# jramapuram/BYOL

Measured on NVIDIA H100. Metric: images/sec, higher is better.
Workload: dtype bf16

## Files before the change

### byol_b200/csrc/common.cuh

```cuda
#pragma once
#include <cuda.h>
#include <cuda_bf16.h>
#include <cuda_runtime.h>
#include <stdint.h>

namespace byol {

typedef __nv_bfloat16 bf16;

void set_last_error(const char* fmt, ...);
int check_launch(const char* what);

static constexpr int kMaxDevices = 64;
int device_slot();
int device_sm_count();

int smem_opt_in(const void* kernel, int bytes, const char* what);

int tmap_bf16(CUtensorMap* tm, const void* base, int rank, const uint64_t* dims, const uint64_t* byte_strides,
              const uint32_t* box, CUtensorMapSwizzle swizzle, const char* what);
int tmap_2d(CUtensorMap* tm, const void* base, uint64_t rows, uint64_t cols, uint64_t ld, uint32_t box_rows,
            uint32_t box_cols, const char* what);

struct Fix128 {
  unsigned long long lo;
  long long hi;
  double spill;
};
static constexpr double kFixSplit = 1048576.0;
Fix128* fix_scratch(cudaStream_t stream, int64_t n);
int fix_done(cudaStream_t stream, int rc);
int fix_flush(Fix128* acc, float* dst, int64_t n, cudaStream_t stream);
int fix_flush_stats(Fix128* acc, float* col_sum, float* col_sqsum, int64_t n, cudaStream_t stream);

__device__ __forceinline__ void fix_add_words(Fix128* acc, unsigned long long lo, long long hi) {
  atomicAdd(&acc->lo, lo);
  atomicAdd(reinterpret_cast<unsigned long long*>(&acc->hi), (unsigned long long)hi);
}
__device__ __forceinline__ void fix_add(Fix128* acc, double v) {
  if (!(fabs(v) < kFixSplit)) {
    const double big = isfinite(v) ? trunc(v * 0x1p-20) * 0x1p20 : v;
    atomicAdd(&acc->spill, big);
    if (!isfinite(v)) return;
    v -= big;
  }
  const double x = v * 0x1p50;
  const double hi = floor(x * 0x1p-32);
  fix_add_words(acc, __double2ull_rn(x - hi * 0x1p32), (long long)hi);
}
__device__ __forceinline__ void fix_add_raw(Fix128* acc, const Fix128& v) {
  fix_add_words(acc, v.lo, v.hi);
  if (v.spill != 0.0) atomicAdd(&acc->spill, v.spill);
}
__host__ __device__ __forceinline__ double fix_value(const Fix128& a) {
  return ((double)a.hi * 0x1p-18 + (double)a.lo * 0x1p-50) + a.spill;
}

#define BYOL_CHECK_ARG(cond, ...)                 \
  do {                                            \
    if (!(cond)) {                                \
      ::byol::set_last_error(__VA_ARGS__);        \
      return -1;                                  \
    }                                             \
  } while (0)

__device__ __forceinline__ uint32_t smem_u32(const void* p) {
  return (uint32_t)__cvta_generic_to_shared(p);
}

__device__ __forceinline__ bool elect_one() {
  uint32_t pred = 0;
  asm volatile(
      "{\n"
      ".reg .b32 %%rx;\n"
      ".reg .pred %%px;\n"
      "elect.sync %%rx|%%px, %1;\n"
      "@%%px mov.s32 %0, 1;\n"
      "}\n"
      : "+r"(pred)
      : "r"(0xffffffffu));
  return pred != 0;
}

__device__ __forceinline__ float warp_sum(float v) {
#pragma unroll
  for (int o = 16; o > 0; o >>= 1) v += __shfl_xor_sync(0xffffffffu, v, o);
  return v;
}

__device__ __forceinline__ void mbar_init(uint64_t* bar, uint32_t count) {
  asm volatile("mbarrier.init.shared::cta.b64 [%0], %1;" ::"r"(smem_u32(bar)), "r"(count) : "memory");
}
__device__ __forceinline__ void fence_mbar_init() {
  asm volatile("fence.mbarrier_init.release.cluster;" ::: "memory");
}
__device__ __forceinline__ void mbar_arrive(uint64_t* bar) {
  asm volatile("mbarrier.arrive.shared::cta.b64 _, [%0];" ::"r"(smem_u32(bar)) : "memory");
}
__device__ __forceinline__ void mbar_arrive_expect_tx(uint64_t* bar, uint32_t bytes) {
  asm volatile("mbarrier.arrive.expect_tx.shared::cta.b64 _, [%0], %1;" ::"r"(smem_u32(bar)), "r"(bytes)
               : "memory");
// ... 98 lines not shown
        "{\n.reg .pred p;\nsetp.ne.b32 p, %98, 0;\n"
        "wgmma.mma_async.sync.aligned.m64n192k16.f32.bf16.bf16 {%0, %1, %2, %3, %4, %5, %6, %7, %8, %9, %10, %11, %12, %13, %14, %15, %16, %17, %18, %19, %20, %21, %22, %23, %24, %25, %26, %27, %28, %29, %30, %31, %32, %33, %34, %35, %36, %37, %38, %39, %40, %41, %42, %43, %44, %45, %46, %47, %48, %49, %50, %51, %52, %53, %54, %55, %56, %57, %58, %59, %60, %61, %62, %63, %64, %65, %66, %67, %68, %69, %70, %71, %72, %73, %74, %75, %76, %77, %78, %79, %80, %81, %82, %83, %84, %85, %86, %87, %88, %89, %90, %91, %92, %93, %94, %95}, %96, %97, p, 1, 1, %99, %100;\n}\n"
        : "+f"(d[0]), "+f"(d[1]), "+f"(d[2]), "+f"(d[3]), "+f"(d[4]), "+f"(d[5]), "+f"(d[6]), "+f"(d[7]), "+f"(d[8]), "+f"(d[9]), "+f"(d[10]), "+f"(d[11]), "+f"(d[12]), "+f"(d[13]), "+f"(d[14]), "+f"(d[15]), "+f"(d[16]), "+f"(d[17]), "+f"(d[18]), "+f"(d[19]), "+f"(d[20]), "+f"(d[21]), "+f"(d[22]), "+f"(d[23]), "+f"(d[24]), "+f"(d[25]), "+f"(d[26]), "+f"(d[27]), "+f"(d[28]), "+f"(d[29]), "+f"(d[30]), "+f"(d[31]), "+f"(d[32]), "+f"(d[33]), "+f"(d[34]), "+f"(d[35]), "+f"(d[36]), "+f"(d[37]), "+f"(d[38]), "+f"(d[39]), "+f"(d[40]), "+f"(d[41]), "+f"(d[42]), "+f"(d[43]), "+f"(d[44]), "+f"(d[45]), "+f"(d[46]), "+f"(d[47]), "+f"(d[48]), "+f"(d[49]), "+f"(d[50]), "+f"(d[51]), "+f"(d[52]), "+f"(d[53]), "+f"(d[54]), "+f"(d[55]), "+f"(d[56]), "+f"(d[57]), "+f"(d[58]), "+f"(d[59]), "+f"(d[60]), "+f"(d[61]), "+f"(d[62]), "+f"(d[63]), "+f"(d[64]), "+f"(d[65]), "+f"(d[66]), "+f"(d[67]), "+f"(d[68]), "+f"(d[69]), "+f"(d[70]), "+f"(d[71]), "+f"(d[72]), "+f"(d[73]), "+f"(d[74]), "+f"(d[75]), "+f"(d[76]), "+f"(d[77]), "+f"(d[78]), "+f"(d[79]), "+f"(d[80]), "+f"(d[81]), "+f"(d[82]), "+f"(d[83]), "+f"(d[84]), "+f"(d[85]), "+f"(d[86]), "+f"(d[87]), "+f"(d[88]), "+f"(d[89]), "+f"(d[90]), "+f"(d[91]), "+f"(d[92]), "+f"(d[93]), "+f"(d[94]), "+f"(d[95])
        : "l"(adesc), "l"(bdesc), "r"(accumulate), "n"(TA), "n"(TB));
  }
  if constexpr (N == 256) {
    asm volatile(
        "{\n.reg .pred p;\nsetp.ne.b32 p, %130, 0;\n"
        "wgmma.mma_async.sync.aligned.m64n256k16.f32.bf16.bf16 {%0, %1, %2, %3, %4, %5, %6, %7, %8, %9, %10, %11, %12, %13, %14, %15, %16, %17, %18, %19, %20, %21, %22, %23, %24, %25, %26, %27, %28, %29, %30, %31, %32, %33, %34, %35, %36, %37, %38, %39, %40, %41, %42, %43, %44, %45, %46, %47, %48, %49, %50, %51, %52, %53, %54, %55, %56, %57, %58, %59, %60, %61, %62, %63, %64, %65, %66, %67, %68, %69, %70, %71, %72, %73, %74, %75, %76, %77, %78, %79, %80, %81, %82, %83, %84, %85, %86, %87, %88, %89, %90, %91, %92, %93, %94, %95, %96, %97, %98, %99, %100, %101, %102, %103, %104, %105, %106, %107, %108, %109, %110, %111, %112, %113, %114, %115, %116, %117, %118, %119, %120, %121, %122, %123, %124, %125, %126, %127}, %128, %129, p, 1, 1, %131, %132;\n}\n"
        : "+f"(d[0]), "+f"(d[1]), "+f"(d[2]), "+f"(d[3]), "+f"(d[4]), "+f"(d[5]), "+f"(d[6]), "+f"(d[7]), "+f"(d[8]), "+f"(d[9]), "+f"(d[10]), "+f"(d[11]), "+f"(d[12]), "+f"(d[13]), "+f"(d[14]), "+f"(d[15]), "+f"(d[16]), "+f"(d[17]), "+f"(d[18]), "+f"(d[19]), "+f"(d[20]), "+f"(d[21]), "+f"(d[22]), "+f"(d[23]), "+f"(d[24]), "+f"(d[25]), "+f"(d[26]), "+f"(d[27]), "+f"(d[28]), "+f"(d[29]), "+f"(d[30]), "+f"(d[31]), "+f"(d[32]), "+f"(d[33]), "+f"(d[34]), "+f"(d[35]), "+f"(d[36]), "+f"(d[37]), "+f"(d[38]), "+f"(d[39]), "+f"(d[40]), "+f"(d[41]), "+f"(d[42]), "+f"(d[43]), "+f"(d[44]), "+f"(d[45]), "+f"(d[46]), "+f"(d[47]), "+f"(d[48]), "+f"(d[49]), "+f"(d[50]), "+f"(d[51]), "+f"(d[52]), "+f"(d[53]), "+f"(d[54]), "+f"(d[55]), "+f"(d[56]), "+f"(d[57]), "+f"(d[58]), "+f"(d[59]), "+f"(d[60]), "+f"(d[61]), "+f"(d[62]), "+f"(d[63]), "+f"(d[64]), "+f"(d[65]), "+f"(d[66]), "+f"(d[67]), "+f"(d[68]), "+f"(d[69]), "+f"(d[70]), "+f"(d[71]), "+f"(d[72]), "+f"(d[73]), "+f"(d[74]), "+f"(d[75]), "+f"(d[76]), "+f"(d[77]), "+f"(d[78]), "+f"(d[79]), "+f"(d[80]), "+f"(d[81]), "+f"(d[82]), "+f"(d[83]), "+f"(d[84]), "+f"(d[85]), "+f"(d[86]), "+f"(d[87]), "+f"(d[88]), "+f"(d[89]), "+f"(d[90]), "+f"(d[91]), "+f"(d[92]), "+f"(d[93]), "+f"(d[94]), "+f"(d[95]), "+f"(d[96]), "+f"(d[97]), "+f"(d[98]), "+f"(d[99]), "+f"(d[100]), "+f"(d[101]), "+f"(d[102]), "+f"(d[103]), "+f"(d[104]), "+f"(d[105]), "+f"(d[106]), "+f"(d[107]), "+f"(d[108]), "+f"(d[109]), "+f"(d[110]), "+f"(d[111]), "+f"(d[112]), "+f"(d[113]), "+f"(d[114]), "+f"(d[115]), "+f"(d[116]), "+f"(d[117]), "+f"(d[118]), "+f"(d[119]), "+f"(d[120]), "+f"(d[121]), "+f"(d[122]), "+f"(d[123]), "+f"(d[124]), "+f"(d[125]), "+f"(d[126]), "+f"(d[127])
        : "l"(adesc), "l"(bdesc), "r"(accumulate), "n"(TA), "n"(TB));
  }
}

template <int N>
__device__ __forceinline__ void acc_store_smem(float* buf, int ld, int row0, int col0, const float (&d)[N / 2]) {
  const int t = threadIdx.x & 127;
  const int r = row0 + (t >> 5) * 16 + ((t & 31) >> 2);
  const int c = col0 + 2 * (t & 3);
#pragma unroll
  for (int j = 0; j < N / 8; ++j) {
    *reinterpret_cast<float2*>(buf + (int64_t)r * ld + c + 8 * j) = make_float2(d[4 * j], d[4 * j + 1]);
    *reinterpret_cast<float2*>(buf + (int64_t)(r + 8) * ld + c + 8 * j) = make_float2(d[4 * j + 2], d[4 * j + 3]);
  }
}
__device__ __forceinline__ void acc_load_row32(const float* src, uint32_t (&r)[32]) {
#pragma unroll
  for (int j = 0; j < 8; ++j) {
    const uint4 q = *reinterpret_cast<const uint4*>(src + 4 * j);
    r[4 * j] = q.x; r[4 * j + 1] = q.y; r[4 * j + 2] = q.z; r[4 * j + 3] = q.w;
  }
}
__host__ __device__ constexpr int acc_ld(int cols) { return cols + 4; }

__device__ __forceinline__ uint64_t make_smem_desc_sw128(uint32_t smem_addr, uint32_t lbo_bytes,
                                                         uint32_t sbo_bytes) {
  uint64_t d = 0;
  d |= (uint64_t)((smem_addr & 0x3FFFFu) >> 4);
  d |= (uint64_t)((lbo_bytes >> 4) & 0x3FFFu) << 16;
  d |= (uint64_t)((sbo_bytes >> 4) & 0x3FFFu) << 32;
  d |= (uint64_t)1 << 62;
  return d;
}

__device__ __forceinline__ uint32_t sw128_offset(uint32_t row, uint32_t chunk) {
  return row * 128u + ((chunk ^ (row & 7u)) << 4);
}

__device__ __forceinline__ uint32_t pack_bf16x2(float lo, float hi) {
  __nv_bfloat162 v = __floats2bfloat162_rn(lo, hi);
  return *reinterpret_cast<uint32_t*>(&v);
}

__device__ __forceinline__ void bulk_load_1d(uint32_t dst_smem, const void* src, uint32_t bytes, uint64_t* bar) {
  asm volatile("cp.async.bulk.shared::cluster.global.mbarrier::complete_tx::bytes [%0], [%1], %2, [%3];" ::"r"(dst_smem),
               "l"(src), "r"(bytes), "r"(smem_u32(bar))
               : "memory");
}
__device__ __forceinline__ void tma_store_3d(const CUtensorMap* tmap, uint32_t src_smem, int c0, int c1, int c2) {
  asm volatile("cp.async.bulk.tensor.3d.global.shared::cta.bulk_group [%0, {%2, %3, %4}], [%1];" ::"l"(tmap),
               "r"(src_smem), "r"(c0), "r"(c1), "r"(c2)
               : "memory");
}

__device__ __forceinline__ uint64_t make_smem_desc_none(uint32_t smem_addr, uint32_t lbo_bytes, uint32_t sbo_bytes) {
  uint64_t d = 0;
  d |= (uint64_t)((smem_addr & 0x3FFFFu) >> 4);
  d |= (uint64_t)((lbo_bytes >> 4) & 0x3FFFu) << 16;
  d |= (uint64_t)((sbo_bytes >> 4) & 0x3FFFu) << 32;
  return d;
}

__device__ __forceinline__ uint64_t f2_pack(uint32_t lo, uint32_t hi) {
  uint64_t r;
  asm("mov.b64 %0, {%1, %2};" : "=l"(r) : "r"(lo), "r"(hi));
  return r;
}
__device__ __forceinline__ float2 f2_unpack(uint64_t v) {
  uint32_t lo, hi;
  asm("mov.b64 {%0, %1}, %2;" : "=r"(lo), "=r"(hi) : "l"(v));
  return make_float2(__uint_as_float(lo), __uint_as_float(hi));
}
__device__ __forceinline__ uint64_t f2_add(uint64_t a, uint64_t b) {
  const float2 x = f2_unpack(a), y = f2_unpack(b);
  return f2_pack(__float_as_uint(x.x + y.x), __float_as_uint(x.y + y.y));
}
__device__ __forceinline__ uint64_t f2_fma(uint64_t a, uint64_t b, uint64_t c) {
  const float2 x = f2_unpack(a), y = f2_unpack(b), z = f2_unpack(c);
  return f2_pack(__float_as_uint(fmaf(x.x, y.x, z.x)), __float_as_uint(fmaf(x.y, y.y, z.y)));
}
__device__ __forceinline__ uint32_t lds32(uint32_t addr) {
  uint32_t w;
  asm volatile("ld.shared.b32 %0, [%1];" : "=r"(w) : "r"(addr));
  return w;
}
__device__ __forceinline__ void stat_acc(uint32_t w, uint64_t& s1, uint64_t& s2) {
  const uint64_t x = f2_pack(w << 16, w & 0xffff0000u);
  s1 = f2_add(s1, x);
  s2 = f2_fma(x, x, s2);
}

__device__ __forceinline__ void stats_narrow(uint32_t stage_base, int lane, int rows_valid, uint64_t& s1,
                                             uint64_t& s2) {
  const uint32_t cp = (uint32_t)lane & 15u, rh = (uint32_t)lane >> 4;
  const uint32_t jc = cp >> 2, wq = cp & 3u;
  uint32_t offq[4];
// ... 20 lines not shown
```

### byol_b200/csrc/conv_igemm.cu

```cuda
#include <stdarg.h>
#include <stdio.h>
#include <stdlib.h>
#include <string.h>

#include "common.cuh"

namespace byol {

static constexpr int BM = 128;
static constexpr int BK = 64;
static constexpr int A_STAGE_BYTES = BM * 128;
static constexpr int GATHER_LAG = 2;

struct ConvGemmParams {
  const bf16* src;
  void* dst;
  const bf16* resid;
  const uint8_t* resid_mask;
  int resid_up;
  const float* resid_f32;
  const float* bias;
  float* col_sum;
  float* col_sqsum;
  Fix128* fx;
  int Nimg, Hs, Ws, C;
  int Ho, Wo;
  int KH, KW;
  int mul, base, dk, div;
  int M, Ndim, Kg;
  int ldc;
  int num_kb;
  int tiles_n;
  int out_fp32;
  int relu;
  int small_src;
  int fold;
  int parity;
  int Hh, Wh;
  int Mc;
  int ncls;
  int cls_list[4];
};

struct TileInfo {
  int m0, n0, nkb;
  int cls_idx, ph, pw, kh0, kw0, nkw;
};

template <bool GROUPED = false>
__device__ __forceinline__ TileInfo tile_info(const ConvGemmParams& p, int tile, int BN_) {
  TileInfo t;
  t.m0 = (tile / p.tiles_n) * BM;
  t.n0 = (tile % p.tiles_n) * BN_;
  t.nkb = p.num_kb;
  t.cls_idx = 0; t.ph = 0; t.pw = 0; t.kh0 = 0; t.kw0 = 0; t.nkw = p.KW;
  if (p.parity) {
    t.cls_idx = t.m0 / p.Mc;
    const int cls = p.cls_list[t.cls_idx];
    t.ph = cls >> 1;
    t.pw = cls & 1;
    t.kh0 = (t.ph + p.base) & 1;
    t.kw0 = (t.pw + p.base) & 1;
    const int nkh = (p.KH - t.kh0 + 1) >> 1;
    t.nkw = (p.KW - t.kw0 + 1) >> 1;
    t.nkb = nkh * t.nkw * (GROUPED ? 1 : p.C / BK);
  }
  return t;
}

template <int BN, int STAGES, bool A_TMA>
struct SmemLayout {
  static constexpr int EW = A_TMA ? 8 : 4;
  static constexpr int CPW = (BN / 32) / (EW / 4);
  static constexpr int NBUF = (A_TMA && BN == 128) ? 1 : 2;
  static constexpr int STAGE_PER_WARP = NBUF * 2048;
  static constexpr int B_STAGE_BYTES = BN * 128;
  static constexpr int A_OFF = 0;
  static constexpr int B_OFF = STAGES * A_STAGE_BYTES;
  static constexpr int STAGE_OUT_OFF = B_OFF + STAGES * B_STAGE_BYTES;
  static constexpr int ACC_LD = acc_ld(BN);
  static constexpr int ACC_OFF = STAGE_OUT_OFF + EW * STAGE_PER_WARP;
  static constexpr int BAR_OFF = ACC_OFF + BM * ACC_LD * 4;
  static constexpr int NEEDED = BAR_OFF + 256;
  static constexpr int TOTAL = NEEDED + 768;
  static_assert(TOTAL <= 232448, "one CTA per SM: <= 227 KB of dynamic shared memory");
};

static constexpr int IG_THREADS = 17 * 32;

template <int BN, int STAGES, bool A_TMA, bool GROUPED = false>
__global__ void __launch_bounds__(IG_THREADS, 1)
conv_igemm_kernel(const __grid_constant__ CUtensorMap tmapA, const __grid_constant__ CUtensorMap tmapB,
                  const __grid_constant__ CUtensorMap tmapC, const ConvGemmParams p, const int num_tiles) {
  static_assert(!GROUPED || (BN == 64 && !A_TMA), "grouped mode: 64-column tiles, gathered A operand");
  using L = SmemLayout<BN, STAGES, A_TMA>;
  constexpr int EW = L::EW;
  constexpr int CPW = L::CPW;
  constexpr int MMA_WARP = 8;
  constexpr int TMA_WARP = MMA_WARP + 8;
  extern __shared__ __align__(1024) uint8_t smem_raw[];
  uint8_t* smem = (uint8_t*)(((uintptr_t)smem_raw + 1023) & ~(uintptr_t)1023);
  if (smem + L::NEEDED > smem_raw + L::TOTAL) __trap();
  uint8_t* smemA = smem + L::A_OFF;
  uint8_t* smemB = smem + L::B_OFF;
  uint64_t* full_bar = (uint64_t*)(smem + L::BAR_OFF);
  uint64_t* empty_bar = full_bar + STAGES;
  uint64_t* tfull_bar = empty_bar + STAGES;
  uint64_t* tempty_bar = tfull_bar + 1;
  uint8_t* stage_out = smem + L::STAGE_OUT_OFF;
  float* accbuf = reinterpret_cast<float*>(smem + L::ACC_OFF);

  const int warp = threadIdx.x >> 5;
  const int lane = threadIdx.x & 31;
  const int num_kb = p.num_kb;

  if (warp == TMA_WARP && lane == 0) {
    for (int s = 0; s < STAGES; ++s) {
      mbar_init(&full_bar[s], A_TMA ? 1u : 129u);
      mbar_init(&empty_bar[s], 2u);
    }
    mbar_init(tfull_bar, 256u);
    mbar_init(tempty_bar, (uint32_t)EW);
    fence_mbar_init();
    tma_prefetch_desc(&tmapB);
    if (A_TMA) tma_prefetch_desc(&tmapA);
    if (!p.out_fp32) tma_prefetch_desc(&tmapC);
  }
  __syncthreads();

  if (warp < EW) {
    const bool do_stats = p.col_sum != nullptr;
    const int quarter = warp & 3;
    const int col_w0 = (warp >> 2) * (CPW * 32);
    const uint32_t stage_base0 = smem_u32(stage_out + warp * L::STAGE_PER_WARP);
    int sbuf = 0;
    constexpr int NACC = CPW;
    uint64_t cs1[NACC], cs2[NACC];
#pragma unroll
    for (int i = 0; i < NACC; ++i) { cs1[i] = 0ull; cs2[i] = 0ull; }
    int local = 0;
    int stat_n0 = -1;
    auto flush_stats = [&]() {
#pragma unroll
      for (int i = 0; i < NACC; ++i) {
        float2 a = f2_unpack(cs1[i]), b = f2_unpack(cs2[i]);
        a.x += __shfl_xor_sync(0xffffffffu, a.x, 16);
        a.y += __shfl_xor_sync(0xffffffffu, a.y, 16);
        b.x += __shfl_xor_sync(0xffffffffu, b.x, 16);
        b.y += __shfl_xor_sync(0xffffffffu, b.y, 16);
        const int col = stat_n0 + col_w0 + i * 32 + 2 * (lane & 15);
        const bool owner = lane < 16;
        if (owner && col < p.Ndim) {
          fix_add(p.fx + col, a.x);
          fix_add(p.fx + col + 1, a.y);
          fix_add(p.fx + p.Ndim + col, b.x);
          fix_add(p.fx + p.Ndim + col + 1, b.y);
        }
        cs1[i] = 0ull; cs2[i] = 0ull;
      }
    };
    for (int tile = blockIdx.x; tile < num_tiles; tile += gridDim.x, ++local) {
      const TileInfo ti = tile_info<GROUPED>(p, tile, BN);
      const int m0 = ti.m0;
      const int n0 = ti.n0;
      if (do_stats && stat_n0 != n0) {
        if (stat_n0 >= 0) flush_stats();
        stat_n0 = n0;
      }
      mbar_wait(tfull_bar, (uint32_t)(local & 1));
      const int mrow0 = m0 + quarter * 32;
      int m = mrow0 + lane;
      const bool mvalid = m < p.M;
      if (p.parity) {
        const int mc = m - ti.cls_idx * p.Mc;
        const int b = mc % p.Wh;
        const int t2 = mc / p.Wh;
        const int a = t2 % p.Hh;
        const int n = t2 / p.Hh;
        m = (n * p.Ho + 2 * a + ti.ph) * p.Wo + 2 * b + ti.pw;
      }
      int rows_valid = p.M - mrow0;
      rows_valid = rows_valid < 0 ? 0 : (rows_valid > 32 ? 32 : rows_valid);
      bool rvalid = mvalid;
      int64_t rrow = m;
      if (p.resid_up) {
        const int w = m % p.Wo;
        const int t2 = m / p.Wo;
        const int h = t2 % p.Ho;
        const int n = t2 / p.Ho;
        rvalid = mvalid && ((h | w) & 1) == 0;
        rrow = ((int64_t)n * (p.Ho >> 1) + (h >> 1)) * (p.Wo >> 1) + (w >> 1);
      }
#pragma unroll
      for (int cl = 0; cl < CPW; ++cl) {
        const int c0 = col_w0 + cl * 32;
        uint32_t r[32];
        acc_load_row32(accbuf + (quarter * 32 + lane) * L::ACC_LD + c0, r);
        if (cl == CPW - 1) {
          __syncwarp();
          if (lane == 0) mbar_arrive(tempty_bar);
        }
        const int nbase = n0 + c0;
        if (nbase >= p.Ndim) continue;
        float v[32];
#pragma unroll
        for (int j = 0; j < 32; ++j) v[j] = __uint_as_float(r[j]);
        if (p.bias != nullptr) {
#pragma unroll
          for (int j = 0; j < 32; ++j)
            if (nbase + j < p.Ndim) v[j] += __ldg(p.bias + nbase + j);
        }
        if (p.resid != nullptr && rvalid) {
          const bf16* rp = p.resid + rrow * p.ldc + nbase;
          const uint8_t* mp = p.resid_mask != nullptr ? p.resid_mask + ((rrow * p.ldc + nbase) >> 3) : nullptr;
#pragma unroll
          for (int j = 0; j < 32; j += 8) {
            if (nbase + j < p.Ndim) {
              uint4 q = *reinterpret_cast<const uint4*>(rp + j);
              const uint32_t mb = mp != nullptr ? (uint32_t)__ldg(mp + (j >> 3)) : 0xffu;
              const __nv_bfloat162* h = reinterpret_cast<const __nv_bfloat162*>(&q);
// ... 24 lines not shown
              if (nbase + j < p.Ndim) {
                uint4 q;
                q.x = pack_bf16x2(v[j], v[j + 1]);
                q.y = pack_bf16x2(v[j + 2], v[j + 3]);
                q.z = pack_bf16x2(v[j + 4], v[j + 5]);
                q.w = pack_bf16x2(v[j + 6], v[j + 7]);
                *reinterpret_cast<uint4*>(op + j) = q;
              }
            }
          }
        } else if (p.out_fp32) {
          if (mvalid) {
            float* op = reinterpret_cast<float*>(p.dst) + (int64_t)m * p.ldc + nbase;
            const bool vec = (p.ldc & 3) == 0;
#pragma unroll
            for (int j = 0; j < 32; j += 4) {
              if (vec && nbase + j + 3 < p.Ndim) {
                *reinterpret_cast<float4*>(op + j) = make_float4(v[j], v[j + 1], v[j + 2], v[j + 3]);
              } else {
#pragma unroll
                for (int e = 0; e < 4; ++e)
                  if (nbase + j + e < p.Ndim) op[j + e] = v[j + e];
              }
            }
          }
        } else {
          const uint32_t stage_base = stage_base0 + (uint32_t)sbuf * 2048u;
          if (lane == 0) { if (L::NBUF == 2) tma_store_wait_read1(); else tma_store_wait_read(); }
          __syncwarp();
#pragma unroll
          for (int j = 0; j < 4; ++j) {
            uint4 q;
            q.x = pack_bf16x2(v[8 * j + 0], v[8 * j + 1]);
            q.y = pack_bf16x2(v[8 * j + 2], v[8 * j + 3]);
            q.z = pack_bf16x2(v[8 * j + 4], v[8 * j + 5]);
            q.w = pack_bf16x2(v[8 * j + 6], v[8 * j + 7]);
            const uint32_t off = (uint32_t)lane * 64u + (uint32_t)((j ^ ((lane >> 1) & 3)) << 4);
            asm volatile("st.shared.v4.b32 [%0], {%1, %2, %3, %4};" ::"r"(stage_base + off), "r"(q.x), "r"(q.y),
                         "r"(q.z), "r"(q.w)
                         : "memory");
          }
          fence_proxy_async_smem();
          __syncwarp();
          if (lane == 0) {
            tma_store_2d(&tmapC, stage_base, nbase, mrow0);
            tma_store_commit();
          }
          if (do_stats) stats_narrow(stage_base, lane, rows_valid, cs1[cl], cs2[cl]);
          if (L::NBUF == 2) sbuf ^= 1;
        }
      }
    }
    if (do_stats && stat_n0 >= 0) flush_stats();
    if (lane == 0) tma_store_wait_all();
  } else if (!A_TMA && warp >= EW && warp < EW + 4) {
    const int tid = threadIdx.x - 128;
    const int chunk = tid & 7;
    const int row0 = tid >> 3;
    int it = 0;
    const bool fast = GROUPED || ((p.C % BK == 0) && (p.KH * p.KW <= 32) && p.small_src);
    for (int tile = blockIdx.x; tile < num_tiles; tile += gridDim.x) {
      const TileInfo ti = tile_info<GROUPED>(p, tile, BN);
      const int m0 = ti.m0;
      if (!GROUPED && p.fold) {
        uint32_t mask[8];
        int roff[8];
#pragma unroll
        for (int i = 0; i < 8; ++i) {
          const int m = m0 + row0 + 16 * i;
          mask[i] = 0u;
          roff[i] = 0;
          if (m < p.M) {
            const int ow = m % p.Wo;
            const int t = m / p.Wo;
            const int oh = t % p.Ho;
            const int n = t / p.Ho;
            const int bh = oh * p.mul + p.base, bw = ow * p.mul + p.base;
            const int sw = bw + chunk;
            roff[i] = ((n * p.Hs + bh) * p.Ws + sw) * 8;
            if (chunk < p.KW && sw >= 0 && sw < p.Ws)
              for (int kh = 0; kh < p.KH; ++kh)
                if (bh + kh >= 0 && bh + kh < p.Hs) mask[i] |= 1u << kh;
          }
        }
        for (int kb = 0; kb < num_kb; ++kb, ++it) {
          const int s = it % STAGES;
          const uint32_t ph = (it / STAGES) & 1;
          if (it >= GATHER_LAG) {
            cp_async_wait<GATHER_LAG - 1>();
            fence_proxy_async_smem();
            mbar_arrive(&full_bar[(it - GATHER_LAG) % STAGES]);
          }
          mbar_wait(&empty_bar[s], ph ^ 1);
          const int tapoff = kb * p.Ws * 8;
          const uint32_t stage_base = smem_u32(smemA + s * A_STAGE_BYTES);
#pragma unroll
          for (int i = 0; i < 8; ++i) {
            const bool v = (mask[i] >> kb) & 1u;
            const bf16* g = v ? p.src + (roff[i] + tapoff) : p.src;
            cp_async16_zfill(stage_base + sw128_offset(row0 + 16 * i, chunk), g, v);
          }
          cp_async_commit();
        }
      } else if (p.parity) {
        uint32_t mask[8];
        int roff[8];
// ... 127 lines not shown
          const int tap = k0 / p.C;
          const int cc = k0 - tap * p.C;
          const int kh = tap / p.KW;
          const int kw = tap - kh * p.KW;
          const int dh = kh * p.dk, dw = kw * p.dk;
          const uint32_t stage_base = smem_u32(smemA + s * A_STAGE_BYTES);
#pragma unroll
          for (int i = 0; i < 8; ++i) {
            int sh = bh[i] + dh, sw = bw[i] + dw;
            bool v = kvalid && sh >= 0 && sw >= 0;
            if (p.div == 2) {
              v = v && ((sh | sw) & 1) == 0;
              sh >>= 1;
              sw >>= 1;
            }
            v = v && sh < p.Hs && sw < p.Ws;
            const bf16* g = v ? p.src + ioff[i] + ((int64_t)sh * p.Ws + sw) * p.C + cc : p.src;
            cp_async16_zfill(stage_base + sw128_offset(row0 + 16 * i, chunk), g, v);
          }
          cp_async_commit();
        }
      }
    }
    cp_async_wait<0>();
    fence_proxy_async_smem();
    for (int j = (it > GATHER_LAG ? it - GATHER_LAG : 0); j < it; ++j) mbar_arrive(&full_bar[j % STAGES]);
  } else if (warp >= MMA_WARP && warp < TMA_WARP) {
    const int wg = (warp - MMA_WARP) >> 2;
    const bool leader = (threadIdx.x & 127) == 0;
    float d[BN / 2];
    int it = 0, local = 0;
    for (int tile = blockIdx.x; tile < num_tiles; tile += gridDim.x, ++local) {
      const int nkb_tile = tile_info<GROUPED>(p, tile, BN).nkb;
      int prev_s = -1;
      for (int kb = 0; kb < nkb_tile; ++kb, ++it) {
        const int s = it % STAGES;
        const uint32_t ph = (it / STAGES) & 1;
        mbar_wait(&full_bar[s], ph);
        const uint64_t adesc = make_smem_desc_sw128(smem_u32(smemA + s * A_STAGE_BYTES + wg * 8192), 16, 1024);
        const uint64_t bdesc = make_smem_desc_sw128(smem_u32(smemB + s * L::B_STAGE_BYTES), 16, 1024);
        wg_fence();
#pragma unroll
        for (int k = 0; k < BK / 16; ++k) {
          wgmma_bf16<BN, 0, 0>(d, adesc + (uint64_t)(2 * k), bdesc + (uint64_t)(2 * k), (uint32_t)((kb | k) != 0));
        }
        wg_commit();
        wg_wait<1>();
        if (leader && prev_s >= 0) mbar_arrive(&empty_bar[prev_s]);
        prev_s = s;
      }
      wg_wait<0>();
      wg_fence_acc(d);
      if (leader && prev_s >= 0) mbar_arrive(&empty_bar[prev_s]);
      mbar_wait(tempty_bar, (uint32_t)((local & 1) ^ 1));
      acc_store_smem<BN>(accbuf, L::ACC_LD, wg * 64, 0, d);
      mbar_arrive(tfull_bar);
    }
  } else if (warp == TMA_WARP) {
    if (lane == 0) {
      constexpr uint32_t tx = (uint32_t)L::B_STAGE_BYTES + (A_TMA ? (uint32_t)A_STAGE_BYTES : 0u);
      int it = 0;
      for (int tile = blockIdx.x; tile < num_tiles; tile += gridDim.x) {
        const TileInfo ti = tile_info<GROUPED>(p, tile, BN);
        const int n0 = ti.n0;
        const int m0 = ti.m0;
        int kh = ti.kh0, kw = ti.kw0, cc = 0;
        for (int kb = 0; kb < ti.nkb; ++kb, ++it) {
          const int s = it % STAGES;
          const uint32_t ph = (it / STAGES) & 1;
          mbar_wait(&empty_bar[s], ph ^ 1);
          mbar_arrive_expect_tx(&full_bar[s], tx);
          int kcol = kb * BK;
          if (p.parity) {
            kcol = (kh * p.KW + kw) * (GROUPED ? BK : p.C) + cc;
            if (!GROUPED) cc += BK;
            if (GROUPED || cc >= p.C) { cc = 0; kw += 2; if (kw >= p.KW) { kw = ti.kw0; kh += 2; } }
          }
          tma_load_2d(smem_u32(smemB + s * L::B_STAGE_BYTES), &tmapB, &full_bar[s], kcol, n0);
          if (A_TMA) tma_load_2d(smem_u32(smemA + s * A_STAGE_BYTES), &tmapA, &full_bar[s], kb * BK, m0);
        }
      }
    }
    __syncwarp();
  }
}

struct WgradParams {
  const bf16* src;
  float* dw;
  int Nimg, Hs, Ws, C;
  int Ho, Wo;
  int KH, KW;
  int stride, pad;
  int M;
  int Cout, Cin_real;
  int tiles_co, tiles_n;
  int splits, kb_per_split, num_kb_total;
  int Cg;
  int groups;
  int fold_kw;
  int small_src;
  Fix128* fx;
  int terms, kb_per_term;
  int ldsrc;
  int dy_term;
  int src_term[6];
};

static constexpr int WG_KROWS = 64;
// ... 165 lines not shown
            const int kwj = (cw + e) >> 3, cj = (cw + e) & 7;
            if (kwj < p.KW && cj < p.Cin_real) add(gp + (int64_t)cj * taps + kwj, e ? v1 : v0);
          }
        } else {
          float* gp = p.dw + ((int64_t)co * p.Cin_real) * taps + group;
          if (cw < p.Cin_real) add(gp + (int64_t)cw * taps, v0);
          if (cw + 1 < p.Cin_real) add(gp + (int64_t)(cw + 1) * taps, v1);
        }
      }
    }
  } else {
    if (lane == 0) {
      constexpr uint32_t tx = (uint32_t)WG_A_STAGE + (B_TMA ? (uint32_t)B_STAGE : 0u);
      for (int it = 0; it < nkb; ++it) {
        const int kb = kb_begin + it;
        const int term = p.terms == 1 ? 0 : kb / p.kb_per_term;
        const int row = (kb - term * p.kb_per_term) * WG_KROWS;
        const int col_a = co0 + term * p.dy_term;
        const int s = it % STAGES;
        const uint32_t ph = (it / STAGES) & 1;
        mbar_wait(&empty_bar[s], ph ^ 1);
        mbar_arrive_expect_tx(&full_bar[s], tx);
        const uint32_t a_base = smem_u32(smemA + s * WG_A_STAGE);
        tma_load_2d(a_base, &tmapA, &full_bar[s], col_a, row);
        tma_load_2d(a_base + WG_KROWS * 128, &tmapA, &full_bar[s], col_a + 64, row);
        if (B_TMA) {
          const uint32_t b_base = smem_u32(smemB + s * B_STAGE);
#pragma unroll
          for (int c = 0; c < NCH; ++c)
            tma_load_2d(b_base + c * (WG_KROWS * 128), &tmapB, &full_bar[s], n0 + 64 * c + p.src_term[term], row);
        }
      }
    }
    __syncwarp();
  }
}

bool gemm_fused_applicable(int M, int C, int Ndim, int ldw, int ldc);
int gemm_fused_launch(const void* src, const void* wt, void* dst, const void* resid, const void* resid_mask,
                      const float* colscale, const float* bias, const float* resid_colscale, void* mask_out,
                      float* col_sum, float* col_sqsum, int M, int C, int Ndim, int ldw, int ldc, int relu, int no_store,
                      int bwd_reduce, cudaStream_t stream);

bool patch_conv_applicable(int H, int W, int C, int Ndim, int KH, int KW, int stride, int pad, int out_fp32,
                           const float* bias, int64_t src_elems);
int patch_conv_launch(const void* src, const void* wt, void* dst, const void* resid, float* col_sum, float* col_sqsum,
                      int Nimg, int H, int W, int C, int Ndim, int ldw, int ldc, int flip, int relu, int sms,
                      cudaStream_t stream, int grouped = 0);

bool patch_wgrad_applicable(int H, int W, int C, int Cin_real, int Cout, int KH, int KW, int stride, int pad);
int patch_wgrad_launch(const void* x, const void* dy, float* dw, int Nimg, int H, int W, int C, int Cout, int sms,
                       cudaStream_t stream, int gs = 0);

template <int BN, int STAGES, bool A_TMA, bool GROUPED = false>
static int launch_igemm(const CUtensorMap& ta, const CUtensorMap& tb, const CUtensorMap& tc,
                        const ConvGemmParams& p, int tiles_m, cudaStream_t stream) {
  using L = SmemLayout<BN, STAGES, A_TMA>;
  auto kern = conv_igemm_kernel<BN, STAGES, A_TMA, GROUPED>;
  if (smem_opt_in((const void*)kern, L::TOTAL, "conv_igemm_kernel") != 0) return -2;
  const int num_tiles = tiles_m * p.tiles_n;
  int grid = device_sm_count();
  if (grid > num_tiles) grid = num_tiles;
  kern<<<grid, IG_THREADS, L::TOTAL, stream>>>(ta, tb, tc, p, num_tiles);
  return check_launch("conv_igemm_kernel");
}

}

using namespace byol;

static int conv_igemm_impl(const void* src, const void* wt, void* dst, const void* resid, const float* resid_f32,
                           const void* resid_mask, int resid_up, const float* bias, float* col_sum, float* col_sqsum,
                           int Nimg, int Hs, int Ws, int C, int Ho, int Wo, int Ndim, int KH, int KW, int stride,
                           int pad, int mode, int ldw, int ldc, int out_fp32, int relu, int force_gather,
                           cudaStream_t stream, int grouped = 0) {
  BYOL_CHECK_ARG(src && wt && dst, "byol_conv_igemm: null pointer");
  BYOL_CHECK_ARG(resid_f32 == nullptr || (out_fp32 && resid == nullptr && !resid_up),
                 "byol_conv_igemm: an fp32 residual needs an fp32 output and no other residual");
  BYOL_CHECK_ARG(C % 8 == 0 && C >= 8, "byol_conv_igemm: C=%d must be a multiple of 8", C);
  BYOL_CHECK_ARG(Ndim > 0 && (Ndim % 8 == 0 || (out_fp32 && resid == nullptr && col_sum == nullptr)),
                 "byol_conv_igemm: Ndim=%d must be a multiple of 8 (any width only for plain fp32 outputs)", Ndim);
  BYOL_CHECK_ARG(ldc >= Ndim && (ldc % 8 == 0 || out_fp32), "byol_conv_igemm: bad ldc=%d", ldc);
  BYOL_CHECK_ARG(!(out_fp32 && col_sum != nullptr), "byol_conv_igemm: fused statistics need a bf16 output");
  BYOL_CHECK_ARG((col_sum == nullptr) == (col_sqsum == nullptr), "byol_conv_igemm: need both statistics or none");
  BYOL_CHECK_ARG(stride == 1 || stride == 2, "byol_conv_igemm: stride %d unsupported", stride);
  BYOL_CHECK_ARG(mode == 0 || mode == 1, "byol_conv_igemm: bad mode %d", mode);
  const int64_t M64 = (int64_t)Nimg * Ho * Wo;
  BYOL_CHECK_ARG(M64 > 0 && M64 < (1ll << 31), "byol_conv_igemm: M out of range");
  BYOL_CHECK_ARG((int64_t)Nimg * Hs * Ws * C < (1ll << 40), "byol_conv_igemm: src too large");
  BYOL_CHECK_ARG(resid_mask == nullptr || (resid != nullptr && ldc % 8 == 0), "byol_conv_igemm: resid_mask without resid");
  BYOL_CHECK_ARG(!resid_up || (resid != nullptr && resid_mask == nullptr && Ho % 2 == 0 && Wo % 2 == 0 &&
                               !(mode == 1 && stride == 2)),
                 "byol_conv_igemm: resid_up needs resid, even output dims and a non-parity mode");
  if (!force_gather && resid_f32 == nullptr && resid != nullptr && !resid_up && KH == 1 && KW == 1 && stride == 1 &&
      pad == 0 && !out_fp32 &&
      col_sum == nullptr && gemm_fused_applicable((int)M64, C, Ndim, ldw, ldc))
    return gemm_fused_launch(src, wt, dst, resid, resid_mask, nullptr, bias, nullptr, nullptr, nullptr, nullptr,
                             (int)M64, C, Ndim, ldw, ldc, relu, 0, 0, stream);
  if (!force_gather && resid_f32 == nullptr && resid_mask == nullptr && !resid_up && Hs == Ho && Ws == Wo &&
      ldw >= 9 * (grouped ? BK : C) &&
      patch_conv_applicable(Hs, Ws, C, Ndim, KH, KW, stride, pad, out_fp32, bias, (int64_t)Nimg * Hs * Ws * C))
    return patch_conv_launch(src, wt, dst, resid, col_sum, col_sqsum, Nimg, Hs, Ws, C, Ndim, ldw, ldc, mode, relu,
                             device_sm_count(), stream, grouped);
  ConvGemmParams p;
  memset(&p, 0, sizeof(p));
  p.src = (const bf16*)src;
  p.dst = dst;
  p.resid = (const bf16*)resid;
  p.resid_mask = (const uint8_t*)resid_mask;
  p.resid_up = resid_up ? 1 : 0;
  p.resid_f32 = resid_f32;
  p.bias = bias;
  p.col_sum = col_sum;
  p.col_sqsum = col_sqsum;
  p.Nimg = Nimg; p.Hs = Hs; p.Ws = Ws; p.C = C; p.Ho = Ho; p.Wo = Wo; p.KH = KH; p.KW = KW;
  if (mode == 0) { p.mul = stride; p.base = -pad; p.dk = 1; p.div = 1; }
  else           { p.mul = 1; p.base = pad; p.dk = -1; p.div = stride; }
  p.M = (int)M64;
  p.Ndim = Ndim;
  p.Kg = KH * KW * (grouped ? BK : C);
  p.fold = (mode == 0 && C == 8 && KW > 1 && KW <= 8 && KH <= 32 && ldw == KH * 64 &&
            (int64_t)Nimg * Hs * Ws * C < (1ll << 31) - (1ll << 24)) ? 1 : 0;
  if (p.fold) p.Kg = KH * 64;
  BYOL_CHECK_ARG(ldw >= p.Kg && ldw % 8 == 0, "byol_conv_igemm: bad ldw=%d (Kg=%d)", ldw, p.Kg);
  p.ldc = ldc;
  p.num_kb = (p.Kg + BK - 1) / BK;
  p.out_fp32 = out_fp32;
  p.relu = relu;
  p.small_src = ((int64_t)Nimg * Hs * Ws * C < (1ll << 31) - (1ll << 24)) ? 1 : 0;
  const int BN = (Ndim > 64 && !grouped) ? 128 : 64;
  p.tiles_n = (Ndim + BN - 1) / BN;
  int tiles_m = (p.M + BM - 1) / BM;
  if (mode == 1 && stride == 2 && Ho % 2 == 0 && Wo % 2 == 0 && C % BK == 0 && p.small_src && KH <= 3 && KW <= 3 &&
      ((int64_t)Nimg * (Ho / 2) * (Wo / 2)) % BM == 0 && !out_fp32) {
    p.parity = 1;
    p.Hh = Ho / 2;
    p.Wh = Wo / 2;
    p.Mc = Nimg * p.Hh * p.Wh;
    p.ncls = 0;
    for (int cls = 0; cls < 4; ++cls) {
      const int ph = cls >> 1, pw = cls & 1;
      const int nkh = (KH - ((ph + pad) & 1) + 1) >> 1, nkw = (KW - ((pw + pad) & 1) + 1) >> 1;
      if (nkh > 0 && nkw > 0) p.cls_list[p.ncls++] = cls;
    }
    if (p.ncls < 4) {
      cudaError_t e = cudaMemsetAsync(dst, 0, (size_t)p.M * ldc * sizeof(bf16), stream);
      if (e != cudaSuccess) { set_last_error("byol_conv_igemm: memset failed: %s", cudaGetErrorString(e)); return -2; }
    }
    tiles_m = p.ncls * (p.Mc / BM);
  }
  const bool a_tma = !force_gather && KH == 1 && KW == 1 && stride == 1 && pad == 0;

  CUtensorMap ta, tb, tc;
  memset(&ta, 0, sizeof(ta));
  if (tmap_2d(&tb, wt, (uint64_t)Ndim, (uint64_t)p.Kg, (uint64_t)ldw, (uint32_t)BN, 64u, "conv_igemm B") != 0) return -3;
  if (!out_fp32) {
    if (tmap_2d(&tc, dst, (uint64_t)p.M, (uint64_t)Ndim, (uint64_t)ldc, 32u, 32u, "conv_igemm C") != 0) return -3;
  } else {
    tc = tb;
  }
  if (a_tma) {
    if (tmap_2d(&ta, src, (uint64_t)p.M, (uint64_t)C, (uint64_t)C, (uint32_t)BM, 64u, "conv_igemm A") != 0) return -3;
  } else {
    ta = tb;
  }
  if (col_sum != nullptr) {
    p.fx = fix_scratch(stream, 2 * (int64_t)Ndim);
    if (p.fx == nullptr) return -2;
  }
  int rc;
  if (grouped) {
    rc = launch_igemm<64, 4, false, true>(ta, tb, tc, p, tiles_m, stream);
  } else if (BN == 128) {
    rc = a_tma ? launch_igemm<128, 3, true>(ta, tb, tc, p, tiles_m, stream)
               : launch_igemm<128, 3, false>(ta, tb, tc, p, tiles_m, stream);
  } else {
    rc = a_tma ? launch_igemm<64, 3, true>(ta, tb, tc, p, tiles_m, stream)
               : launch_igemm<64, 4, false>(ta, tb, tc, p, tiles_m, stream);
  }
  if (rc != 0 || col_sum == nullptr) return rc;
  return fix_flush_stats(p.fx, col_sum, col_sqsum, Ndim, stream);
}

extern "C" int byol_conv_igemm(const void* src, const void* wt, void* dst, const void* resid,
                               const void* resid_mask, int resid_up, const float* bias, float* col_sum, float* col_sqsum, int Nimg, int Hs, int Ws, int C, int Ho, int Wo,
                               int Ndim, int KH, int KW, int stride, int pad, int mode, int ldw, int ldc,
                               int out_fp32, int relu, int force_gather, cudaStream_t stream) {
  return conv_igemm_impl(src, wt, dst, resid, nullptr, resid_mask, resid_up, bias, col_sum, col_sqsum, Nimg, Hs, Ws, C,
                         Ho, Wo, Ndim, KH, KW, stride, pad, mode, ldw, ldc, out_fp32, relu, force_gather, stream);
}

static bool grouped_geometry_ok(const char* what, int Nimg, int H, int W, int C, int Ho, int Wo, int KH, int KW,
                                int stride, int pad) {
  if (Nimg <= 0 || H <= 0 || W <= 0 || C < 64 || C % 64 != 0 || KH != 3 || KW != 3 || pad != 1 ||
      (stride != 1 && stride != 2) || Ho != (H - 1) / stride + 1 || Wo != (W - 1) / stride + 1) {
    set_last_error("%s: unsupported geometry (N=%d H=%d W=%d C=%d Ho=%d Wo=%d KH=%d KW=%d stride=%d pad=%d): needs "
                   "C %% 64 == 0, 3x3, pad 1, stride 1 or 2", what, Nimg, H, W, C, Ho, Wo, KH, KW, stride, pad);
    return false;
  }
  const int64_t big = (int64_t)Nimg * (H > Ho ? H : Ho) * (W > Wo ? W : Wo) * C;
  if (big >= (1ll << 31) - (1ll << 24)) {
    set_last_error("%s: tensor of %lld elements too large for 32-bit offsets", what, (long long)big);
    return false;
  }
  return true;
}

extern "C" int byol_conv_fprop_grouped(const void* x, const void* wt, void* y, float* col_sum, float* col_sqsum,
                                       int Nimg, int H, int W, int C, int Ho, int Wo, int KH, int KW, int stride,
                                       int pad, cudaStream_t stream) {
  BYOL_CHECK_ARG(x && wt && y, "byol_conv_fprop_grouped: null pointer");
  if (!grouped_geometry_ok("byol_conv_fprop_grouped", Nimg, H, W, C, Ho, Wo, KH, KW, stride, pad)) return -1;
  return conv_igemm_impl(x, wt, y, nullptr, nullptr, nullptr, 0, nullptr, col_sum, col_sqsum, Nimg, H, W, C, Ho, Wo,
                         C, KH, KW, stride, pad, 0, KH * KW * BK, C, 0, 0, 0, stream, 1);
}

extern "C" int byol_conv_dgrad_grouped(const void* dy, const void* wd, void* dx, int Nimg, int Ho, int Wo, int C,
                                       int H, int W, int KH, int KW, int stride, int pad, cudaStream_t stream) {
  BYOL_CHECK_ARG(dy && wd && dx, "byol_conv_dgrad_grouped: null pointer");
  if (!grouped_geometry_ok("byol_conv_dgrad_grouped", Nimg, H, W, C, Ho, Wo, KH, KW, stride, pad)) return -1;
  return conv_igemm_impl(dy, wd, dx, nullptr, nullptr, nullptr, 0, nullptr, nullptr, nullptr, Nimg, Ho, Wo, C, H, W,
                         C, KH, KW, stride, pad, 1, KH * KW * BK, C, 0, 0, 0, stream, 1);
}

extern "C" int byol_conv_dgrad_planes(const void* dy, const void* wd, float* dx, const float* resid_f32, int Nimg,
                                      int Hs, int Ws, int Cout, int H, int W, int Cin, int KH, int KW, int stride,
                                      int pad, int T, cudaStream_t stream) {
  BYOL_CHECK_ARG((T == 3 || T == 6) && Cout % 8 == 0 && Cin % 8 == 0, "byol_conv_dgrad_planes: bad args (T=%d Cout=%d Cin=%d)",
                 T, Cout, Cin);
  return conv_igemm_impl(dy, wd, dx, nullptr, resid_f32, nullptr, 0, nullptr, nullptr, nullptr, Nimg, Hs, Ws, T * Cout,
                         H, W, Cin, KH, KW, stride, pad, 1, KH * KW * T * Cout, Cin, 1, 0, 0, stream);
// ... 111 lines not shown
```

Measured before the change: 2244.

## Hand off bf16 accumulator tiles via stmatrix double buffer for plain 1x1 convs

For plain 1x1 conv GEMMs with no bias, residual or relu, the MMA warpgroups now convert accumulators to bf16 and write them with stmatrix into a double-buffered, 64B-swizzled output tile. Epilogue warps then TMA-store that tile directly and compute column stats from it, so the fp32 staging buffer and its single-buffer handshake are gone. Per-column statistics are also accumulated in shared-memory fixed-point words before one global atomic flush per CTA, which cuts global atomic traffic. This adds a new template path and more shared memory, and stats are now computed from bf16-rounded values instead of fp32.

```diff
diff --git a/byol_b200/csrc/common.cuh b/byol_b200/csrc/common.cuh
--- a/byol_b200/csrc/common.cuh
+++ b/byol_b200/csrc/common.cuh
@@ -37,16 +37,35 @@
   atomicAdd(&acc->lo, lo);
   atomicAdd(reinterpret_cast<unsigned long long*>(&acc->hi), (unsigned long long)hi);
 }
-__device__ __forceinline__ void fix_add(Fix128* acc, double v) {
+__device__ __forceinline__ bool fix_take_spill(Fix128* acc, double& v) {
   if (!(fabs(v) < kFixSplit)) {
     const double big = isfinite(v) ? trunc(v * 0x1p-20) * 0x1p20 : v;
     atomicAdd(&acc->spill, big);
-    if (!isfinite(v)) return;
+    if (!isfinite(v)) return false;
     v -= big;
   }
+  return true;
+}
+__device__ __forceinline__ void fix_words(double v, unsigned long long& lo, long long& hi) {
   const double x = v * 0x1p50;
-  const double hi = floor(x * 0x1p-32);
-  fix_add_words(acc, __double2ull_rn(x - hi * 0x1p32), (long long)hi);
+  const double h = floor(x * 0x1p-32);
+  lo = __double2ull_rn(x - h * 0x1p32);
+  hi = (long long)h;
+}
+__device__ __forceinline__ void fix_add(Fix128* acc, double v) {
+  if (!fix_take_spill(acc, v)) return;
+  unsigned long long lo;
+  long long hi;
+  fix_words(v, lo, hi);
+  fix_add_words(acc, lo, hi);
+}
+__device__ __forceinline__ void fix_add_local(Fix128* acc, unsigned long long* words, double v) {
+  if (!fix_take_spill(acc, v)) return;
+  unsigned long long lo;
+  long long hi;
+  fix_words(v, lo, hi);
+  atomicAdd(&words[0], lo);
+  atomicAdd(&words[1], (unsigned long long)hi);
 }
 __device__ __forceinline__ void fix_add_raw(Fix128* acc, const Fix128& v) {
   fix_add_words(acc, v.lo, v.hi);
@@ -251,6 +270,29 @@
   return *reinterpret_cast<uint32_t*>(&v);
 }
 
+__device__ __forceinline__ void stmatrix_x4(uint32_t addr, uint32_t r0, uint32_t r1, uint32_t r2, uint32_t r3) {
+  asm volatile("stmatrix.sync.aligned.m8n8.x4.shared.b16 [%0], {%1, %2, %3, %4};" ::"r"(addr), "r"(r0), "r"(r1),
+               "r"(r2), "r"(r3)
+               : "memory");
+}
+
+template <int N>
+__device__ __forceinline__ void acc_store_bf16_sw64(uint32_t base, const float (&d)[N / 2]) {
+  const int t = threadIdx.x & 127;
+  const int warp = t >> 5, lane = t & 31;
+  const uint32_t r = (uint32_t)(16 * (warp & 1) + 8 * ((lane >> 3) & 1) + (lane & 7));
+  const uint32_t rbase = base + (uint32_t)(warp >> 1) * (N / 32) * 2048u + r * 64u;
+  const uint32_t sw = (r >> 1) & 3u;
+  const uint32_t gh = (uint32_t)lane >> 4;
+#pragma unroll
+  for (int p = 0; p < N / 16; ++p) {
+    const uint32_t g = 2u * (uint32_t)p + gh;
+    stmatrix_x4(rbase + (g >> 2) * 2048u + (((g & 3u) ^ sw) << 4), pack_bf16x2(d[8 * p], d[8 * p + 1]),
+                pack_bf16x2(d[8 * p + 2], d[8 * p + 3]), pack_bf16x2(d[8 * p + 4], d[8 * p + 5]),
+                pack_bf16x2(d[8 * p + 6], d[8 * p + 7]));
+  }
+}
+
 __device__ __forceinline__ void bulk_load_1d(uint32_t dst_smem, const void* src, uint32_t bytes, uint64_t* bar) {
   asm volatile("cp.async.bulk.shared::cluster.global.mbarrier::complete_tx::bytes [%0], [%1], %2, [%3];" ::"r"(dst_smem),
                "l"(src), "r"(bytes), "r"(smem_u32(bar))
diff --git a/byol_b200/csrc/conv_igemm.cu b/byol_b200/csrc/conv_igemm.cu
--- a/byol_b200/csrc/conv_igemm.cu
+++ b/byol_b200/csrc/conv_igemm.cu
@@ -34,6 +34,7 @@
   int out_fp32;
   int relu;
   int small_src;
+  int local_stats;
   int fold;
   int parity;
   int Hh, Wh;
@@ -68,7 +69,7 @@
   return t;
 }
 
-template <int BN, int STAGES, bool A_TMA>
+template <int BN, int STAGES, bool A_TMA, bool H16 = false>
 struct SmemLayout {
   static constexpr int EW = A_TMA ? 8 : 4;
   static constexpr int CPW = (BN / 32) / (EW / 4);
@@ -80,7 +81,8 @@
   static constexpr int STAGE_OUT_OFF = B_OFF + STAGES * B_STAGE_BYTES;
   static constexpr int ACC_LD = acc_ld(BN);
   static constexpr int ACC_OFF = STAGE_OUT_OFF + EW * STAGE_PER_WARP;
-  static constexpr int BAR_OFF = ACC_OFF + BM * ACC_LD * 4;
+  static constexpr int OUT_TILE_BYTES = BM * BN * 2;
+  static constexpr int BAR_OFF = H16 ? STAGE_OUT_OFF + 2 * OUT_TILE_BYTES : ACC_OFF + BM * ACC_LD * 4;
   static constexpr int NEEDED = BAR_OFF + 256;
   static constexpr int TOTAL = NEEDED + 768;
   static_assert(TOTAL <= 232448, "one CTA per SM: <= 227 KB of dynamic shared memory");
@@ -88,12 +90,15 @@
 
 static constexpr int IG_THREADS = 17 * 32;
 
-template <int BN, int STAGES, bool A_TMA, bool GROUPED = false>
+__device__ __forceinline__ void epilogue_bar_sync(int n) { asm volatile("bar.sync 1, %0;" ::"r"(n) : "memory"); }
+
+template <int BN, int STAGES, bool A_TMA, bool GROUPED = false, bool H16 = false>
 __global__ void __launch_bounds__(IG_THREADS, 1)
 conv_igemm_kernel(const __grid_constant__ CUtensorMap tmapA, const __grid_constant__ CUtensorMap tmapB,
                   const __grid_constant__ CUtensorMap tmapC, const ConvGemmParams p, const int num_tiles) {
   static_assert(!GROUPED || (BN == 64 && !A_TMA), "grouped mode: 64-column tiles, gathered A operand");
-  using L = SmemLayout<BN, STAGES, A_TMA>;
+  static_assert(!H16 || A_TMA, "bf16 hand-off: plain GEMM only (no parity mode)");
+  using L = SmemLayout<BN, STAGES, A_TMA, H16>;
   constexpr int EW = L::EW;
   constexpr int CPW = L::CPW;
   constexpr int MMA_WARP = 8;
@@ -107,6 +112,8 @@
   uint64_t* empty_bar = full_bar + STAGES;
   uint64_t* tfull_bar = empty_bar + STAGES;
   uint64_t* tempty_bar = tfull_bar + 1;
+  uint64_t* ofull_bar = tempty_bar + 1;
+  uint64_t* oempty_bar = ofull_bar + 2;
   uint8_t* stage_out = smem + L::STAGE_OUT_OFF;
   float* accbuf = reinterpret_cast<float*>(smem + L::ACC_OFF);
 
@@ -121,6 +128,10 @@
     }
     mbar_init(tfull_bar, 256u);
     mbar_init(tempty_bar, (uint32_t)EW);
+    for (int b = 0; b < 2; ++b) {
+      mbar_init(&ofull_bar[b], 256u);
+      mbar_init(&oempty_bar[b], (uint32_t)EW);
+    }
     fence_mbar_init();
     tma_prefetch_desc(&tmapB);
     if (A_TMA) tma_prefetch_desc(&tmapA);
@@ -140,6 +151,12 @@
     for (int i = 0; i < NACC; ++i) { cs1[i] = 0ull; cs2[i] = 0ull; }
     int local = 0;
     int stat_n0 = -1;
+    const bool local_stats = H16 && do_stats && p.local_stats;
+    unsigned long long* lstats = reinterpret_cast<unsigned long long*>(smem + L::NEEDED);
+    if (local_stats) {
+      for (int i = threadIdx.x; i < 4 * p.Ndim; i += EW * 32) lstats[i] = 0ull;
+      epilogue_bar_sync(EW * 32);
+    }
     auto flush_stats = [&]() {
 #pragma unroll
       for (int i = 0; i < NACC; ++i) {
@@ -150,7 +167,12 @@
         b.y += __shfl_xor_sync(0xffffffffu, b.y, 16);
         const int col = stat_n0 + col_w0 + i * 32 + 2 * (lane & 15);
         const bool owner = lane < 16;
-        if (owner && col < p.Ndim) {
+        if (owner && col < p.Ndim && local_stats) {
+          fix_add_local(p.fx + col, lstats + 2 * col, a.x);
+          fix_add_local(p.fx + col + 1, lstats + 2 * (col + 1), a.y);
+          fix_add_local(p.fx + p.Ndim + col, lstats + 2 * (p.Ndim + col), b.x);
+          fix_add_local(p.fx + p.Ndim + col + 1, lstats + 2 * (p.Ndim + col + 1), b.y);
+        } else if (owner && col < p.Ndim) {
           fix_add(p.fx + col, a.x);
           fix_add(p.fx + col + 1, a.y);
           fix_add(p.fx + p.Ndim + col, b.x);
@@ -166,6 +188,30 @@
       if (do_stats && stat_n0 != n0) {
         if (stat_n0 >= 0) flush_stats();
         stat_n0 = n0;
+      }
+      if constexpr (H16) {
+        const int buf = local & 1;
+        mbar_wait(&ofull_bar[buf], (uint32_t)((local >> 1) & 1));
+        const int mrow0 = m0 + quarter * 32;
+        int rows_valid = p.M - mrow0;
+        rows_valid = rows_valid < 0 ? 0 : (rows_valid > 32 ? 32 : rows_valid);
+        const uint32_t qbase = smem_u32(stage_out + buf * L::OUT_TILE_BYTES) + (uint32_t)quarter * (BN / 32) * 2048u;
+#pragma unroll
+        for (int cl = 0; cl < CPW; ++cl) {
+          const int c0 = col_w0 + cl * 32;
+          const int nbase = n0 + c0;
+          if (nbase >= p.Ndim) continue;
+          const uint32_t blk = qbase + (uint32_t)(c0 / 32) * 2048u;
+          if (lane == 0) {
+            tma_store_2d(&tmapC, blk, nbase, mrow0);
+            tma_store_commit();
+          }
+          if (do_stats) stats_narrow(blk, lane, rows_valid, cs1[cl], cs2[cl]);
+        }
+        if (lane == 0) tma_store_wait_read();
+        __syncwarp();
+        if (lane == 0) mbar_arrive(&oempty_bar[buf]);
+        continue;
       }
       mbar_wait(tfull_bar, (uint32_t)(local & 1));
       const int mrow0 = m0 + quarter * 32;
@@ -296,6 +342,13 @@
       }
     }
     if (do_stats && stat_n0 >= 0) flush_stats();
+    if (local_stats) {
+      epilogue_bar_sync(EW * 32);
+      for (int i = threadIdx.x; i < 2 * p.Ndim; i += EW * 32) {
+        const unsigned long long lo = lstats[2 * i], hi = lstats[2 * i + 1];
+        if ((lo | hi) != 0ull) fix_add_words(p.fx + i, lo, (long long)hi);
+      }
+    }
     if (lane == 0) tma_store_wait_all();
   } else if (!A_TMA && warp >= EW && warp < EW + 4) {
     const int tid = threadIdx.x - 128;
@@ -529,9 +582,17 @@
       wg_wait<0>();
       wg_fence_acc(d);
       if (leader && prev_s >= 0) mbar_arrive(&empty_bar[prev_s]);
-      mbar_wait(tempty_bar, (uint32_t)((local & 1) ^ 1));
-      acc_store_smem<BN>(accbuf, L::ACC_LD, wg * 64, 0, d);
-      mbar_arrive(tfull_bar);
+      if constexpr (H16) {
+        const int buf = local & 1;
+        mbar_wait(&oempty_bar[buf], (uint32_t)(((local >> 1) & 1) ^ 1));
+        acc_store_bf16_sw64<BN>(smem_u32(stage_out + buf * L::OUT_TILE_BYTES) + (uint32_t)wg * 2 * (BN / 32) * 2048u, d);
+        fence_proxy_async_smem();
+        mbar_arrive(&ofull_bar[buf]);
+      } else {
+        mbar_wait(tempty_bar, (uint32_t)((local & 1) ^ 1));
+        acc_store_smem<BN>(accbuf, L::ACC_LD, wg * 64, 0, d);
+        mbar_arrive(tfull_bar);
+      }
     }
   } else if (warp == TMA_WARP) {
     if (lane == 0) {
@@ -803,16 +864,20 @@
 int patch_wgrad_launch(const void* x, const void* dy, float* dw, int Nimg, int H, int W, int C, int Cout, int sms,
                        cudaStream_t stream, int gs = 0);
 
-template <int BN, int STAGES, bool A_TMA, bool GROUPED = false>
+template <int BN, int STAGES, bool A_TMA, bool GROUPED = false, bool H16 = false>
 static int launch_igemm(const CUtensorMap& ta, const CUtensorMap& tb, const CUtensorMap& tc,
                         const ConvGemmParams& p, int tiles_m, cudaStream_t stream) {
-  using L = SmemLayout<BN, STAGES, A_TMA>;
-  auto kern = conv_igemm_kernel<BN, STAGES, A_TMA, GROUPED>;
-  if (smem_opt_in((const void*)kern, L::TOTAL, "conv_igemm_kernel") != 0) return -2;
+  using L = SmemLayout<BN, STAGES, A_TMA, H16>;
+  auto kern = conv_igemm_kernel<BN, STAGES, A_TMA, GROUPED, H16>;
+  ConvGemmParams q = p;
+  const int64_t local_bytes = 32 * (int64_t)p.Ndim;
+  q.local_stats = (H16 && p.col_sum != nullptr && L::TOTAL + local_bytes <= 232448) ? 1 : 0;
+  const int smem = L::TOTAL + (q.local_stats ? (int)local_bytes : 0);
+  if (smem_opt_in((const void*)kern, smem, "conv_igemm_kernel") != 0) return -2;
   const int num_tiles = tiles_m * p.tiles_n;
   int grid = device_sm_count();
   if (grid > num_tiles) grid = num_tiles;
-  kern<<<grid, IG_THREADS, L::TOTAL, stream>>>(ta, tb, tc, p, num_tiles);
+  kern<<<grid, IG_THREADS, smem, stream>>>(ta, tb, tc, q, num_tiles);
   return check_launch("conv_igemm_kernel");
 }
 
@@ -901,6 +966,8 @@
     tiles_m = p.ncls * (p.Mc / BM);
   }
   const bool a_tma = !force_gather && KH == 1 && KW == 1 && stride == 1 && pad == 0;
+  const bool h16 = a_tma && !out_fp32 && bias == nullptr && resid == nullptr && resid_mask == nullptr &&
+                   resid_f32 == nullptr && !relu;
 
   CUtensorMap ta, tb, tc;
   memset(&ta, 0, sizeof(ta));
@@ -923,11 +990,13 @@
   if (grouped) {
     rc = launch_igemm<64, 4, false, true>(ta, tb, tc, p, tiles_m, stream);
   } else if (BN == 128) {
-    rc = a_tma ? launch_igemm<128, 3, true>(ta, tb, tc, p, tiles_m, stream)
-               : launch_igemm<128, 3, false>(ta, tb, tc, p, tiles_m, stream);
+    rc = h16     ? launch_igemm<128, 3, true, false, true>(ta, tb, tc, p, tiles_m, stream)
+         : a_tma ? launch_igemm<128, 3, true>(ta, tb, tc, p, tiles_m, stream)
+                 : launch_igemm<128, 3, false>(ta, tb, tc, p, tiles_m, stream);
   } else {
-    rc = a_tma ? launch_igemm<64, 3, true>(ta, tb, tc, p, tiles_m, stream)
-               : launch_igemm<64, 4, false>(ta, tb, tc, p, tiles_m, stream);
+    rc = h16     ? launch_igemm<64, 3, true, false, true>(ta, tb, tc, p, tiles_m, stream)
+         : a_tma ? launch_igemm<64, 3, true>(ta, tb, tc, p, tiles_m, stream)
+                 : launch_igemm<64, 4, false>(ta, tb, tc, p, tiles_m, stream);
   }
   if (rc != 0 || col_sum == nullptr) return rc;
   return fix_flush_stats(p.fx, col_sum, col_sqsum, Ndim, stream);
```

Result: faster. 2318, median of 6 (+3.3%).
